# schmidtjonathan/Climate2Weather

Measured on AMD Instinct MI355X. Metric: UNet denoise steps/sec (train fwd+bwd+allreduce+AdamW+EMA windows/s), higher is better.
Workload: dtype bf16; 1 GPU; configs/sda_unet.yml default net, 5 vars x window 13 = 65 ch, 128x128, bf16 training step, 128 windows/GPU/step; global_batch=128, parallelism=dp1, params=72132929

## Files before the change

### climate2weather_amd/csrc/wgrad_patch.hip

```cpp
#include <algorithm>
#include <cstdint>
#include <cstdlib>
#include <utility>
#include "conv_geom.h"

#include "knobs.h"
#include "launch.h"


namespace {

constexpr int NTHREADS = 512;
constexpr int KPX = 128;
constexpr int ABYTES = KPX * 256;
constexpr int PPITCH = 24;
constexpr int NPIECE = 10 * 3;
constexpr int PBYTES = NPIECE * 1024;
constexpr int NSLOT_A = 3, NSLOT_P = 2;
constexpr int PBASE = NSLOT_A * ABYTES;
constexpr int LDS_BYTES = PBASE + NSLOT_P * PBYTES;

struct WpArgs {
    const void* dy;
    const void* x;
    float* dw;
    float* db;
    int B, H, W, Cin, Cout, ldy;
    int up;
    int ktiles, ktiles_per_split;
    float* ws;
    int direct;
    float* wsb;
    int det;
};

struct WpItem {
    const void* dy;
    const void* x;
    float* dw;
    float* db;
};
constexpr int WP_MAX_ITEMS = 16;
struct WpGroupArgs {
    WpArgs c;
    int n;
    int live_per_item;
    unsigned long long ws_item_floats;
    unsigned long long wsb_item_floats;
    WpItem item[WP_MAX_ITEMS];
};



__device__ __forceinline__ uint32_t sel_oob(bool ok, uint32_t v) {
    asm volatile("" : "+v"(v));
    return ok ? v : C2W_OOB;
}

__device__ __forceinline__ uint32_t swzA(int row) { return (uint32_t)(((row & 3) << 2) | ((row >> 2) & 3)); }
__device__ __forceinline__ uint32_t swzP(int pix) { return (uint32_t)((((pix >> 1) & 1) << 1) | (((pix >> 3) & 1) << 2)); }

__device__ __forceinline__ int wp_xcd_order(int bid, int nblk) {
    const int xcd = bid & 7, q = nblk >> 3, r = nblk & 7;
    return (xcd < r ? xcd * (q + 1) : r * (q + 1) + (xcd - r) * q) + (bid >> 3);
}

template <typename T, bool PAIR = false, bool NARROW = false>
__device__ __forceinline__ void wgrad_patch_body(const WpArgs& p, const int L) {
    constexpr int ESZ = sizeof(T);
    constexpr bool BF = ESZ == 2;
    constexpr int COT = 256 / ESZ;
    constexpr int CIB = 128 / ESZ;
    constexpr int MTW = BF ? 4 : 1;
    extern __shared__ __attribute__((aligned(16))) char smem[];

    const int tid = threadIdx.x, lane = tid & 63;
    const int wid = __builtin_amdgcn_readfirstlane(tid >> 6);
    const int li = lane & 15, lg = lane >> 4;
    static_assert(!NARROW || (BF && !PAIR), "narrow-M form: 16-bit, 16-pixel-wide tiles");
    const int mt0 = BF ? (NARROW ? (wid >> 2) * 4 : (wid & 1) * 4) : (wid >> 1);
    const int nt = BF ? (NARROW ? (wid & 3) : (wid >> 1)) : (wid & 1);
    const bool light = NARROW && wid >= 4;

    const int ncib = p.Cin / CIB;
    const int tilesM = (p.Cout + COT - 1) / COT;
    const int tilesMN = tilesM * ncib;
    const int split = L / tilesMN, mn = L - split * tilesMN;
    const int tm = mn / ncib, cb = mn - tm * ncib;
    const int co0 = tm * COT, ci0 = cb * CIB;
    const int H = p.H, W = p.W;
    const int tw = PAIR ? 1 : W >> 4, tpi = (H >> 3) * tw;
    const int t0 = split * p.ktiles_per_split;
    const int t1 = (t0 + p.ktiles_per_split < p.ktiles) ? t0 + p.ktiles_per_split : p.ktiles;

    const int Ws = p.up ? W >> 1 : W;
    const size_t ximg = (size_t)(p.up ? (H >> 1) * Ws : H * W) * p.Cin * ESZ;
    const size_t yimg = (size_t)H * W * p.ldy * ESZ;
    const uint32_t a_step = PAIR ? (uint32_t)(16 * p.ldy * ESZ) : (uint32_t)(2 * W * p.ldy * ESZ);
    auto dy_voff0 = [&](int tid_) -> uint32_t {
        const int row = tid_ >> 4, pc = tid_ & 15;
        const uint32_t lc = (uint32_t)pc ^ swzA(row);
        const int c = co0 + (int)lc * (16 / ESZ);
        if constexpr (PAIR) {
            return sel_oob(c < p.Cout, (uint32_t)((((row >> 4) * 8 + (row & 7)) * p.ldy + c) * ESZ) + (uint32_t)((row >> 3) & 1) * (uint32_t)yimg);
        } else {
            return sel_oob(c < p.Cout, (uint32_t)((((row >> 4) * W + (row & 15)) * p.ldy + c) * ESZ));
        }
    };
    auto patch_piece = [&](int r) -> int {
        const int pc = r * 8 + wid;
        return pc < NPIECE ? pc : NPIECE - 1;
    };
    auto patch_voff = [&](int r, int lane_, int oh0, int ow0) -> uint32_t {
        const int pc = patch_piece(r);
        const int pr = pc / 3, pg = pc - pr * 3;
        const int px = pg * 8 + (lane_ >> 3);
        const uint32_t lanepart = (uint32_t)(((lane_ & 7) ^ swzP(pr * PPITCH + px)) << 4) + (uint32_t)ci0 * ESZ;
        if constexpr (PAIR) {
            const int pimg = px >= 10 ? 1 : 0;
            const int ih = pr - 1, iw = px - 1 - 10 * pimg;
            const bool ok = (unsigned)ih < 8u && (unsigned)iw < 8u && px < 20;
            return sel_oob(ok, (uint32_t)((ih * 8 + iw) * p.Cin) * ESZ + (uint32_t)pimg * (uint32_t)(64 * p.Cin * ESZ) + lanepart);
        } else {
            const int ih = oh0 - 1 + pr, iw = ow0 - 1 + px;
            const bool ok = (unsigned)ih < (unsigned)H && (unsigned)iw < (unsigned)W && px < 18;
            const int spix = p.up ? (ih >> 1) * Ws + (iw >> 1) : ih * W + iw;
            return sel_oob(ok, (uint32_t)(spix * p.Cin) * ESZ + lanepart);
        }
    };

    auto tile_origin = [&](int t, int& b, int& oh0, int& ow0) {
        b = PAIR ? 2 * t : t / tpi;
        const int tt = PAIR ? 0 : t - (t / tpi) * tpi;
        const int ty = tt / tw, tx = tt - ty * tw;
        b = __builtin_amdgcn_readfirstlane(b);
        oh0 = __builtin_amdgcn_readfirstlane(ty << 3);
        ow0 = __builtin_amdgcn_readfirstlane(tx << 4);
    };
    struct TileSrc {
        __amdgpu_buffer_rsrc_t rsrc;
        int oh0, ow0;
        uint32_t aso;
        char* base;
    };
    auto srcA = [&](int t, int sa) {
        int b, oh0, ow0;
        tile_origin(t, b, oh0, ow0);
        const uint32_t nimg = PAIR && b + 1 < p.B ? 2u : 1u;
        TileSrc s;
        s.rsrc = make_rsrc((const char*)p.dy + (size_t)b * yimg, (uint32_t)yimg * nimg);
        s.oh0 = oh0;
        s.ow0 = ow0;
        s.aso = (uint32_t)((oh0 * W + ow0) * p.ldy) * ESZ;
        s.base = smem + sa * ABYTES + wid * 1024;
        return s;
    };
    auto srcP = [&](int t, int sp) {
        int b, oh0, ow0;
        tile_origin(t, b, oh0, ow0);
        const uint32_t nimg = PAIR && b + 1 < p.B ? 2u : 1u;
        TileSrc s;
        s.rsrc = make_rsrc((const char*)p.x + (size_t)b * ximg, (uint32_t)ximg * nimg);
        s.oh0 = oh0;
        s.ow0 = ow0;
        s.aso = 0;
        s.base = smem + PBASE + sp * PBYTES;
        return s;
    };
    auto pieceA = [&](const TileSrc& s, int i, bool live = true) {
        int tid_ = tid;
        asm volatile("" : "+v"(tid_));
        const uint32_t v = dy_voff0(tid_);
        glds16(s.rsrc, s.base + i * 8192, sel_oob(live, v), s.aso + (uint32_t)i * a_step);
    };
    auto pieceP = [&](const TileSrc& s, int r, bool live = true) {
        int lane_ = lane;
        asm volatile("" : "+v"(lane_));
        const uint32_t v = patch_voff(r, lane_, s.oh0, s.ow0);
        glds16(s.rsrc, s.base + patch_piece(r) * 1024, sel_oob(live, v), 0);
    };
    auto issueA = [&](int t, int sa) {
        const TileSrc s = srcA(t, sa);
#pragma unroll
        for (int i = 0; i < 4; ++i) pieceA(s, i);
    };
    auto issueP = [&](int t, int sp) {
        const TileSrc s = srcP(t, sp);
#pragma unroll
        for (int r = 0; r < 4; ++r) pieceP(s, r);
    };

    f32x4_t acc[9][MTW];
#pragma unroll
    for (int t = 0; t < 9; ++t)
#pragma unroll
        for (int m = 0; m < MTW; ++m) acc[t][m] = (f32x4_t){0.f, 0.f, 0.f, 0.f};
    const bool do_bias = p.db != nullptr && cb == 0 && nt == 0;
    f32x4_t accb[MTW];
#pragma unroll
    for (int m = 0; m < MTW; ++m) accb[m] = (f32x4_t){0.f, 0.f, 0.f, 0.f};

    uint32_t offA[MTW][2], offB[9][2];
    if constexpr (BF) {
        const int qq = li >> 2, pp = li & 3;
#pragma unroll
        for (int h = 0; h < 2; ++h) {
            const int row = 8 * lg + qq + 4 * h;
            const uint32_t f = swzA(row);
#pragma unroll
            for (int m = 0; m < MTW; ++m)
                offA[m][h] = (uint32_t)(row * 256 + (((((mt0 + m) * 2 + (pp >> 1)) ^ f) & 15) << 4) + 8 * (pp & 1));
            const int r = lg >> 1, c = 8 * (lg & 1) + qq + 4 * h;
#pragma unroll
            for (int t = 0; t < 9; ++t) {
                const int pix = (r + t / 3) * PPITCH + c + t % 3 + (PAIR ? 2 * (lg & 1) : 0);
                offB[t][h] = (uint32_t)(pix * 128 + (((uint32_t)(nt * 2 + (pp >> 1)) ^ swzP(pix)) << 4) + 8 * (pp & 1));
            }
        }
    }

    if (t0 < t1) {
        issueP(t0, 0);
        issueA(t0, 0);
        const TileSrc s1 = srcA(t0 + 1 < t1 ? t0 + 1 : t0, 1);
#pragma unroll
        for (int i = 0; i < 4; ++i) pieceA(s1, i, t0 + 1 < t1);
    }
    int sa = 0, sp = 0;
    for (int t = t0; t < t1; ++t) {
        asm volatile("s_waitcnt vmcnt(4)" ::: "memory");
        __builtin_amdgcn_s_barrier();
        const bool hasP = t + 1 < t1, hasA = t + 2 < t1;
        const TileSrc nP = srcP(hasP ? t + 1 : t, sp ^ 1), nA = srcA(hasA ? t + 2 : t, sa == 0 ? 2 : sa - 1);
        if constexpr (!BF) {
#pragma unroll
            for (int r = 0; r < 4; ++r) pieceP(nP, r, hasP);
#pragma unroll
            for (int i = 0; i < 4; ++i) pieceA(nA, i, hasA);
        }
        const char* const SA = smem + sa * ABYTES;
        const char* const SP = smem + PBASE + sp * PBYTES;
        if constexpr (BF) {
            const uint32_t sA = (uint32_t)(uintptr_t)SA, sP = (uint32_t)(uintptr_t)SP;
            auto rd = [&](tr_frag& f, uint32_t base, uint32_t o0, uint32_t o1, auto IMMc) {
                constexpr int IMM = decltype(IMMc)::value;
                asm volatile("ds_read_b64_tr_b16 %0, %1 offset:%2" : "=v"(f.lo) : "v"(base + o0), "n"(IMM));
                asm volatile("ds_read_b64_tr_b16 %0, %1 offset:%2" : "=v"(f.hi) : "v"(base + o1), "n"(IMM));
            };
            static_for<4>([&](auto KSc) {
                constexpr int ks = decltype(KSc)::value;
                {
                    const bool first = wid < 4;
                    if ((ks == 0 && first) || (ks == 1 && !first)) {
#pragma unroll
                        for (int r = 0; r < 4; ++r) pieceP(nP, r, hasP);
                    }
                    if ((ks == 2 && first) || (ks == 3 && !first)) {
#pragma unroll
                        for (int i = 0; i < 4; ++i) pieceA(nA, i, hasA);
                    }
                }
                constexpr int PF = 2;
                tr_frag a[MTW], bq[PF + 1];
                rd(a[0], sA, offA[0][0], offA[0][1], IC<ks * 32 * 256>{});
                if (!light) {
#pragma unroll
                    for (int m = 1; m < MTW; ++m) rd(a[m], sA, offA[m][0], offA[m][1], IC<ks * 32 * 256>{});
                }
                static_for<PF>([&](auto Jc) {
                    constexpr int j = decltype(Jc)::value;
                    rd(bq[j], sP, offB[j][0], offB[j][1], IC<ks * 2 * PPITCH * 128>{});
                });
                static_for<9>([&](auto TPc) {
                    constexpr int tp = decltype(TPc)::value;
                    if constexpr (tp + PF < 9) rd(bq[(tp + PF) % (PF + 1)], sP, offB[tp + PF][0], offB[tp + PF][1], IC<ks * 2 * PPITCH * 128>{});
                    constexpr int AHEAD = (tp + PF < 9 ? PF : 8 - tp) * 2;
                    if constexpr (AHEAD == 4) asm volatile("s_waitcnt lgkmcnt(4)" ::: "memory");
                    else if constexpr (AHEAD == 2) asm volatile("s_waitcnt lgkmcnt(2)" ::: "memory");
                    else asm volatile("s_waitcnt lgkmcnt(0)" ::: "memory");
                    __builtin_amdgcn_sched_barrier(0);
                    const bf16x8_t bfr = bq[tp % (PF + 1)].vec();
                    acc[tp][0] = mfma16s<T>(a[0].vec(), bfr, acc[tp][0]);
                    if (!light) {
#pragma unroll
                        for (int m = 1; m < MTW; ++m) acc[tp][m] = mfma16s<T>(a[m].vec(), bfr, acc[tp][m]);
                    }
                    if (tp == 8 && do_bias) {
                        const bf16x8_t ones = __builtin_bit_cast(bf16x8_t, ones16<T>());
                        accb[0] = mfma16s<T>(a[0].vec(), ones, accb[0]);
                        if (!light) {
#pragma unroll
                            for (int m = 1; m < MTW; ++m) accb[m] = mfma16s<T>(a[m].vec(), ones, accb[m]);
                        }
                    }
                    __builtin_amdgcn_sched_barrier(0);
                });
            });
        } else {
#pragma unroll 4
            for (int kk = 0; kk < 32; ++kk) {
                const int row = kk * 4 + lg;
                const float a = *(const float*)(SA + row * 256 + ((((uint32_t)(mt0 * 4 + (li >> 2))) ^ swzA(row)) << 4) + (li & 3) * 4);
                const int r = kk >> 2, c = 4 * (kk & 3) + lg;
#pragma unroll
                for (int tp = 0; tp < 9; ++tp) {
                    const int pix = (r + tp / 3) * PPITCH + c + tp % 3 + (PAIR && (kk & 2) ? 2 : 0);
                    const float bv = *(const float*)(SP + pix * 128 + ((((uint32_t)(nt * 4 + (li >> 2))) ^ swzP(pix)) << 4) + (li & 3) * 4);
                    acc[tp][0] = __builtin_amdgcn_mfma_f32_16x16x4f32(a, bv, acc[tp][0], 0, 0, 0);
                }
                if (do_bias) accb[0] = __builtin_amdgcn_mfma_f32_16x16x4f32(a, 1.0f, accb[0], 0, 0, 0);
            }
        }
        sa = sa == 2 ? 0 : sa + 1;
        sp ^= 1;
    }

    if (t0 >= t1) return;
    if (do_bias && li == 0) {
#pragma unroll
        for (int m = 0; m < MTW; ++m)
#pragma unroll
            for (int r = 0; r < 4; ++r) {
                const int row = (mt0 + m) * 16 + lg * 4 + r;
                const int co = co0 + row;
                if (p.det) {
                    if (p.wsb != nullptr) p.wsb[((size_t)split * tilesM + tm) * COT + row] = accb[m][r];
                    else if (co < p.Cout) p.db[co] = p.db[co] + accb[m][r];
                } else if (co < p.Cout) {
                    atomicAdd(p.db + co, accb[m][r]);
                }
            }
    }
    constexpr int OS = CIB + 4;
    float* const O = (float*)smem;
#pragma unroll
    for (int tp = 0; tp < 9; ++tp) {
        __syncthreads();
#pragma unroll
        for (int m = 0; m < MTW; ++m)
#pragma unroll
            for (int r = 0; r < 4; ++r) O[((mt0 + m) * 16 + lg * 4 + r) * OS + nt * 16 + li] = acc[tp][m][r];
        __syncthreads();
        if (p.ws != nullptr) {
            float* const dst = p.ws + (((size_t)split * tilesMN + mn) * 9 + tp) * (COT * CIB);
            for (int idx = tid; idx < COT * CIB; idx += NTHREADS) dst[idx] = O[(idx / CIB) * OS + (idx % CIB)];
        } else if (p.direct) {
            for (int idx = tid; idx < COT * CIB; idx += NTHREADS) {
                const int row = idx / CIB, col = idx - row * CIB;
                const int co = co0 + row;
                if (co < p.Cout) {
                    float* const d = p.dw + ((size_t)co * 9 + tp) * p.Cin + ci0 + col;
                    *d = *d + O[row * OS + col];
                }
            }
        } else {
            for (int idx = tid; idx < COT * CIB; idx += NTHREADS) {
                const int row = idx / CIB, col = idx - row * CIB;
                const int co = co0 + row;
                if (co < p.Cout) atomicAdd(p.dw + ((size_t)co * 9 + tp) * p.Cin + ci0 + col, O[row * OS + col]);
            }
        }
    }
}

template <typename T, bool PAIR = false, bool NARROW = false>
__global__ __launch_bounds__(NTHREADS, 2) void wgrad_patch_kernel(const WpArgs p) {
    wgrad_patch_body<T, PAIR, NARROW>(p, wp_xcd_order((int)blockIdx.x, (int)gridDim.x));
}

typedef __attribute__((address_space(4))) const char wp_kernarg_t;
__device__ __forceinline__ WpItem wp_item(int it) {
    const WpItem __attribute__((address_space(4)))* tab =
        (const WpItem __attribute__((address_space(4)))*)((wp_kernarg_t*)__builtin_amdgcn_kernarg_segment_ptr() + offsetof(WpGroupArgs, item));
    WpItem r;
    r.dy = tab[it].dy;
    r.x = tab[it].x;
    r.dw = tab[it].dw;
    r.db = tab[it].db;
    return r;
}

template <typename T, bool PAIR = false>
__global__ __launch_bounds__(NTHREADS, 2) void wgrad_patch_group_kernel(const WpGroupArgs g) {
    const int Lg = wp_xcd_order((int)blockIdx.x, (int)gridDim.x);
    const int it = __builtin_amdgcn_readfirstlane(Lg / g.live_per_item);
    const int L = Lg - it * g.live_per_item;
    const WpItem e = wp_item(it);
    WpArgs p = g.c;
    p.dy = e.dy;
    p.x = e.x;
    p.dw = e.dw;
    p.db = e.db;
    p.ws = g.c.ws != nullptr ? g.c.ws + (size_t)it * g.ws_item_floats : nullptr;
    p.wsb = g.c.wsb != nullptr ? g.c.wsb + (size_t)it * g.wsb_item_floats : nullptr;
    wgrad_patch_body<T, PAIR, false>(p, L);
}

struct WgradBiasReduce {
    const float* wsb;
    float* db;
    int cols, tpo, nmain;
};
static inline WgradBiasReduce bias_reduce_of(const float* wsb, float* db, int cols, int nsplit, int nmain) {
    WgradBiasReduce br;
    br.wsb = wsb; br.db = db; br.cols = cols; br.tpo = det_reduce_tpo(nsplit); br.nmain = nmain;
    return br;
}

#ifndef C2W_RED_COLS
#define C2W_RED_COLS 64
#endif
template <int COT, int CIB>
__device__ __forceinline__ void wgrad_reduce_body(const float* __restrict__ ws, float* __restrict__ dw, int nsplit, int tilesMN, int ncib,
                                                  int Cin, int Cout, int nblk) {
    constexpr int RC = C2W_RED_COLS, RG = 256 / RC;
    __shared__ f32x4_t red[RG][RC];
    const size_t per4 = (size_t)tilesMN * 9 * COT * CIB / 4;
    const f32x4_t* ws4 = (const f32x4_t*)ws;
    const int q = threadIdx.x % RC, grp = threadIdx.x / RC;
    for (size_t base = (size_t)blockIdx.x * RC; base < per4; base += (size_t)nblk * RC) {
        const size_t i4 = base + q;
        f32x4_t acc = {0.f, 0.f, 0.f, 0.f};
        if (i4 < per4) {
#pragma unroll 8
            for (int sidx = grp; sidx < nsplit; sidx += RG) acc += ws4[(size_t)sidx * per4 + i4];
        }
        red[grp][q] = acc;
        __syncthreads();
        if (grp == 0 && i4 < per4) {
#pragma unroll
            for (int g2 = 1; g2 < RG; ++g2) acc += red[g2][q];
            const size_t i = i4 * 4;
            const int col = (int)(i % CIB);
            size_t r = i / CIB;
            const int row = (int)(r % COT);
            r /= COT;
            const int tp = (int)(r % 9);
            const int mn = (int)(r / 9);
            const int tm = mn / ncib, cb = mn - tm * ncib;
            const int co = tm * COT + row;
            if (co < Cout) {
                f32x4_t* d = (f32x4_t*)(dw + ((size_t)co * 9 + tp) * Cin + cb * CIB + col);
                *d = *d + acc;
            }
        }
        __syncthreads();
    }
}

template <int COT, int CIB>
__global__ __launch_bounds__(256) void wgrad_reduce_kernel(const float* __restrict__ ws, float* __restrict__ dw, int nsplit, int tilesMN, int ncib,
                                                           int Cin, int Cout, WgradBiasReduce br) {
    if ((int)blockIdx.x >= br.nmain) {
        det_reduce_body(br.wsb, br.db, nsplit, Cout, Cout, 0, br.tpo, br.cols, (int)blockIdx.x - br.nmain);
        return;
    }
    wgrad_reduce_body<COT, CIB>(ws, dw, nsplit, tilesMN, ncib, Cin, Cout, br.nmain);
}
template <int COT, int CIB>
__global__ __launch_bounds__(256) void wgrad_reduce_group_kernel(const WpGroupArgs g, int nsplit, int tilesMN, int ncib, WgradBiasReduce br) {
    const int it = (int)blockIdx.y;
    const WpItem e = wp_item(it);
    if ((int)blockIdx.x >= br.nmain) {
        if (e.db != nullptr)
            det_reduce_body(g.c.wsb + (size_t)it * g.wsb_item_floats, e.db, nsplit, g.c.Cout, g.c.Cout, 0, br.tpo, br.cols, (int)blockIdx.x - br.nmain);
        return;
    }
    wgrad_reduce_body<COT, CIB>(g.c.ws + (size_t)it * g.ws_item_floats, e.dw, nsplit, tilesMN, ncib, g.c.Cin, g.c.Cout, br.nmain);
}

template <int ESZ, bool PAIR>
static void split_plan(const C2wConvArgs& a, int& ktiles, int& tilesMN, int& nsplit, int& ktiles_per_split) {
    constexpr int COT = 256 / ESZ, CIB = 128 / ESZ;
    ktiles = PAIR ? ((a.B + 1) >> 1) * (a.Hout >> 3) : a.B * (a.Hout >> 3) * (a.Wout >> 4);
    tilesMN = ((a.Cout + COT - 1) / COT) * (a.Cin / CIB);
    nsplit = c2w_cu_count() / tilesMN;
    if (nsplit > ktiles) nsplit = ktiles;
    if (nsplit < 1) nsplit = 1;
    ktiles_per_split = (ktiles + nsplit - 1) / nsplit;
    nsplit = (ktiles + ktiles_per_split - 1) / ktiles_per_split;
}

template <int ESZ, bool PAIR>
static size_t ws_need(const C2wConvArgs& a) {
    constexpr int COT = 256 / ESZ, CIB = 128 / ESZ;
    int ktiles, tilesMN, nsplit, per;
    split_plan<ESZ, PAIR>(a, ktiles, tilesMN, nsplit, per);
    const size_t bias_rows = (a.flags & C2W_CONV_DETERMINISTIC) ? (size_t)nsplit * ((a.Cout + COT - 1) / COT) * COT * sizeof(float) : 0;
    return nsplit > 1 ? (size_t)nsplit * tilesMN * 9 * COT * CIB * sizeof(float) + bias_rows : 0;
}

template <typename T, bool PAIR, bool NARROW = false>
int launch(const C2wConvArgs& a, float* dw, float* db, float* ws, size_t ws_bytes, hipStream_t st) {
    constexpr int ESZ = sizeof(T);
    constexpr int COT = 256 / ESZ, CIB = 128 / ESZ;
    WpArgs p;
    p.dy = a.y; p.x = a.x; p.dw = dw; p.db = db;
    p.B = a.B; p.H = a.Hout; p.W = a.Wout; p.Cin = a.Cin; p.Cout = a.Cout; p.ldy = a.ldy;
    p.up = a.mode == C2W_CONV_UP ? 1 : 0;
    int tilesMN, nsplit;
    split_plan<ESZ, PAIR>(a, p.ktiles, tilesMN, nsplit, p.ktiles_per_split);
    if (int rc = c2w_lds_optin<wgrad_patch_kernel<T, PAIR, NARROW>>(LDS_BYTES)) return rc;
    const size_t need = (size_t)nsplit * tilesMN * 9 * COT * CIB * sizeof(float);
    const int bias_cols = (tilesMN / (a.Cin / CIB)) * COT;
    p.det = (a.flags & C2W_CONV_DETERMINISTIC) ? 1 : 0;
    if (p.det) {
        if (c2w_knobs().wgrad_atomics) return C2W_ERR_BAD_ARG;
        if (nsplit > 1 && (ws == nullptr || need + (size_t)nsplit * bias_cols * sizeof(float) > ws_bytes)) return C2W_ERR_BAD_ARG;
    }
    p.ws = (ws != nullptr && need <= ws_bytes && nsplit > 1 && !c2w_knobs().wgrad_atomics) ? ws : nullptr;
    p.wsb = p.det && nsplit > 1 && db != nullptr ? ws + need / sizeof(float) : nullptr;
    p.direct = nsplit == 1 && !c2w_knobs().wgrad_atomics ? 1 : 0;
    wgrad_patch_kernel<T, PAIR, NARROW><<<tilesMN * nsplit, NTHREADS, LDS_BYTES, st>>>(p);
    if (p.ws != nullptr) {
        const size_t per_split = (size_t)tilesMN * 9 * COT * CIB;
        const int grid = (int)std::min<size_t>((per_split / 4 + C2W_RED_COLS - 1) / C2W_RED_COLS, 8192);
        const int extra = p.wsb != nullptr ? det_reduce_blocks(nsplit, a.Cout) : 0;
        wgrad_reduce_kernel<COT, CIB><<<grid + extra, 256, 0, st>>>(p.ws, dw, nsplit, tilesMN, a.Cin / CIB, a.Cin, a.Cout,
                                                                    bias_reduce_of(p.wsb, db, bias_cols, nsplit, grid));
    }
    return (int)hipGetLastError();
}

static void group_plan(int n, int tilesMN, int ktiles, int& nsplit, int& ktiles_per_split) {
    const int T = n * tilesMN, cus = c2w_cu_count();
    double best = 1e30;
    nsplit = 1;
    for (int r = 0; r <= 4; ++r) {
        int ns = r == 0 ? 1 : (cus * r) / T;
        if (ns < 1) ns = 1;
        if (ns > ktiles) ns = ktiles;
        const int per = (ktiles + ns - 1) / ns;
        ns = (ktiles + per - 1) / per;
        const int rounds = (T * ns + cus - 1) / cus;
        const double cost = rounds * (per * 4.1 + (ns > 1 ? 28.0 : 16.0)) + (ns > 1 ? 10.0 : 0.0);
        if (cost < best - 1e-9) {
            best = cost;
            nsplit = ns;
        }
    }
    ktiles_per_split = (ktiles + nsplit - 1) / nsplit;
}

template <int ESZ, bool PAIR>
static size_t group_ws_need(const C2wConvArgs& a, int n) {
    constexpr int COT = 256 / ESZ, CIB = 128 / ESZ;
    int ktiles, tilesMN, ns1, per1, nsplit, per;
    split_plan<ESZ, PAIR>(a, ktiles, tilesMN, ns1, per1);
    group_plan(n, tilesMN, ktiles, nsplit, per);
    const size_t bias_rows = (a.flags & C2W_CONV_DETERMINISTIC) ? (size_t)n * nsplit * ((a.Cout + COT - 1) / COT) * COT * sizeof(float) : 0;
    return nsplit > 1 ? (size_t)n * nsplit * tilesMN * 9 * COT * CIB * sizeof(float) + bias_rows : 0;
}

template <typename T, bool PAIR>
int launch_group(const C2wConvArgs& a, const C2wWgradItem* items, int n, float* ws, size_t ws_bytes, hipStream_t st) {
    constexpr int ESZ = sizeof(T);
    constexpr int COT = 256 / ESZ, CIB = 128 / ESZ;
    WpGroupArgs g;
    WpArgs& p = g.c;
    p.dy = nullptr; p.x = nullptr; p.dw = nullptr; p.db = nullptr;
    p.B = a.B; p.H = a.Hout; p.W = a.Wout; p.Cin = a.Cin; p.Cout = a.Cout; p.ldy = a.ldy;
    p.up = a.mode == C2W_CONV_UP ? 1 : 0;
    int tilesMN, ns1, per1, nsplit;
    split_plan<ESZ, PAIR>(a, p.ktiles, tilesMN, ns1, per1);
    group_plan(n, tilesMN, p.ktiles, nsplit, p.ktiles_per_split);
    const size_t item_floats = (size_t)nsplit * tilesMN * 9 * COT * CIB;
    const int bias_cols = (tilesMN / (a.Cin / CIB)) * COT;
    p.det = (a.flags & C2W_CONV_DETERMINISTIC) ? 1 : 0;
    const size_t bias_item_floats = p.det ? (size_t)nsplit * bias_cols : 0;
    if (nsplit > 1 && (ws == nullptr || (size_t)n * (item_floats + bias_item_floats) * sizeof(float) > ws_bytes)) return C2W_ERR_BAD_ARG;
    p.ws = nsplit > 1 ? ws : nullptr;
    p.wsb = p.det && nsplit > 1 ? ws + (size_t)n * item_floats : nullptr;
    g.wsb_item_floats = bias_item_floats;
    p.direct = nsplit == 1 ? 1 : 0;
    g.n = n;
    g.live_per_item = tilesMN * nsplit;
    g.ws_item_floats = item_floats;
    for (int i = 0; i < WP_MAX_ITEMS; ++i) {
        const C2wWgradItem& e = items[i < n ? i : n - 1];
        g.item[i].dy = e.dy; g.item[i].x = e.x; g.item[i].dw = e.dw; g.item[i].db = e.dbias;
    }
    if (int rc = c2w_lds_optin<wgrad_patch_group_kernel<T, PAIR>>(LDS_BYTES)) return rc;
    wgrad_patch_group_kernel<T, PAIR><<<g.live_per_item * n, NTHREADS, LDS_BYTES, st>>>(g);
    if (p.ws != nullptr) {
        const size_t per_split = (size_t)tilesMN * 9 * COT * CIB;
        const int grid = (int)std::min<size_t>((per_split / 4 + C2W_RED_COLS - 1) / C2W_RED_COLS, 8192);
        const int extra = p.wsb != nullptr ? det_reduce_blocks(nsplit, a.Cout) : 0;
        wgrad_reduce_group_kernel<COT, CIB><<<dim3(grid + extra, n), 256, 0, st>>>(g, nsplit, tilesMN, a.Cin / CIB,
                                                                                   bias_reduce_of(p.wsb, nullptr, bias_cols, nsplit, grid));
    }
    return (int)hipGetLastError();
}

}

bool c2w_wgrad_patch_group_eligible(const C2wConvArgs& a, int n, int dtype) {
    const bool narrow = dtype != C2W_DTYPE_F32 && !c2w_wgrad_patch_pair(a) && a.Cout <= 80;
    return c2w_wgrad_patch_eligible(a) && n >= 2 && n <= WP_MAX_ITEMS && !narrow && !c2w_knobs().wgrad_atomics;
}

int c2w_wgrad_patch_group(const C2wConvArgs& a, const C2wWgradItem* items, int n, float* ws, size_t ws_bytes, int dtype, hipStream_t st) {
    if (c2w_wgrad_patch_pair(a)) return c2w_by_dtype(dtype, [&](auto t) { return launch_group<decltype(t), true>(a, items, n, ws, ws_bytes, st); });
    return c2w_by_dtype(dtype, [&](auto t) { return launch_group<decltype(t), false>(a, items, n, ws, ws_bytes, st); });
}

size_t c2w_wgrad_patch_group_ws_bytes(const C2wConvArgs& a, int n, int dtype) {
    const bool pair = c2w_wgrad_patch_pair(a);
    if (dtype == C2W_DTYPE_F32) return pair ? group_ws_need<4, true>(a, n) : group_ws_need<4, false>(a, n);
    return pair ? group_ws_need<2, true>(a, n) : group_ws_need<2, false>(a, n);
}

bool c2w_wgrad_patch_pair(const C2wConvArgs& a) {
    return a.mode == C2W_CONV_S1 && a.Win == 8 && a.Hin == 8;
}

bool c2w_wgrad_patch_eligible(const C2wConvArgs& a) {
    if (a.mode == C2W_CONV_UP)
        return a.Hout == 2 * a.Hin && a.Wout == 2 * a.Win && (a.Hout & 7) == 0 && (a.Wout & 15) == 0;
    return a.mode == C2W_CONV_S1 && a.Hin == a.Hout && a.Win == a.Wout && (a.Hin & 7) == 0 && ((a.Win & 15) == 0 || c2w_wgrad_patch_pair(a));
}

int c2w_wgrad_patch(const C2wConvArgs& a, float* dw, float* db, float* ws, size_t ws_bytes, int dtype, hipStream_t st) {
    if (c2w_wgrad_patch_pair(a)) return c2w_by_dtype(dtype, [&](auto t) { return launch<decltype(t), true>(a, dw, db, ws, ws_bytes, st); });
    if (dtype != C2W_DTYPE_F32 && a.Cout <= 80)
        return c2w_by_dtype16(dtype, [&](auto t) { return launch<decltype(t), false, true>(a, dw, db, ws, ws_bytes, st); });
    return c2w_by_dtype(dtype, [&](auto t) { return launch<decltype(t), false>(a, dw, db, ws, ws_bytes, st); });
}

size_t c2w_wgrad_patch_ws_bytes(const C2wConvArgs& a, int dtype) {
    const bool pair = c2w_wgrad_patch_pair(a);
    if (dtype == C2W_DTYPE_F32) return pair ? ws_need<4, true>(a) : ws_need<4, false>(a);
    return pair ? ws_need<2, true>(a) : ws_need<2, false>(a);
}
```

Baseline: 2802 windows/s.

## Spread wgrad bias MFMAs across waves and add flat split-K reduce path

Moves bias-gradient accumulation off a single wave. Each wave in the bf16 path now computes at most one 16-row bias tile, and the M-tile order is rotated per wave so that different waves own different tiles. The light path zeros the unused wsb rows. A second, independent change adds a grid-stride flat reduction kernel for split-K workspaces when nsplit is at most 32. It uses several independent accumulators and a smaller grid sized from the CU count, replacing the column-block reduce body. Risks are wrong bias coverage if the ownership mapping misses tiles, and lower parallelism in the reduce for large outputs.

After: 2824 windows/s, median of 6. No clear change (+0.8%).

```diff
diff --git a/climate2weather_amd/csrc/wgrad_patch.hip b/climate2weather_amd/csrc/wgrad_patch.hip
--- a/climate2weather_amd/csrc/wgrad_patch.hip
+++ b/climate2weather_amd/csrc/wgrad_patch.hip
@@ -195,10 +195,16 @@
     for (int t = 0; t < 9; ++t)
 #pragma unroll
         for (int m = 0; m < MTW; ++m) acc[t][m] = (f32x4_t){0.f, 0.f, 0.f, 0.f};
-    const bool do_bias = p.db != nullptr && cb == 0 && nt == 0;
-    f32x4_t accb[MTW];
-#pragma unroll
-    for (int m = 0; m < MTW; ++m) accb[m] = (f32x4_t){0.f, 0.f, 0.f, 0.f};
+    const int rot = BF && !light ? nt : 0;
+    auto tile_of = [&](int m) { return mt0 + ((m + rot) & (MTW - 1)); };
+    int bm = -1;
+    if (p.db != nullptr) {
+        const int half2 = ncib >= 2 ? 1 : 0;
+        if constexpr (!BF) bm = cb == 0 && nt == 0 ? 0 : -1;
+        else if (light) bm = cb == half2 && nt == 0 ? 0 : -1;
+        else bm = cb == (half2 ? nt >> 1 : 0) ? nt : -1;
+    }
+    f32x4_t accb = (f32x4_t){0.f, 0.f, 0.f, 0.f};
 
     uint32_t offA[MTW][2], offB[9][2];
     if constexpr (BF) {
@@ -209,7 +215,7 @@
             const uint32_t f = swzA(row);
 #pragma unroll
             for (int m = 0; m < MTW; ++m)
-                offA[m][h] = (uint32_t)(row * 256 + (((((mt0 + m) * 2 + (pp >> 1)) ^ f) & 15) << 4) + 8 * (pp & 1));
+                offA[m][h] = (uint32_t)(row * 256 + ((((tile_of(m) * 2 + (pp >> 1)) ^ f) & 15) << 4) + 8 * (pp & 1));
             const int r = lg >> 1, c = 8 * (lg & 1) + qq + 4 * h;
 #pragma unroll
             for (int t = 0; t < 9; ++t) {
@@ -285,13 +291,9 @@
 #pragma unroll
                         for (int m = 1; m < MTW; ++m) acc[tp][m] = mfma16s<T>(a[m].vec(), bfr, acc[tp][m]);
                     }
-                    if (tp == 8 && do_bias) {
+                    if (tp == 8 && bm >= 0) {
                         const bf16x8_t ones = __builtin_bit_cast(bf16x8_t, ones16<T>());
-                        accb[0] = mfma16s<T>(a[0].vec(), ones, accb[0]);
-                        if (!light) {
-#pragma unroll
-                            for (int m = 1; m < MTW; ++m) accb[m] = mfma16s<T>(a[m].vec(), ones, accb[m]);
-                        }
+                        accb = mfma16s<T>(a[0].vec(), ones, accb);
                     }
                     __builtin_amdgcn_sched_barrier(0);
                 });
@@ -308,7 +310,7 @@
                     const float bv = *(const float*)(SP + pix * 128 + ((((uint32_t)(nt * 4 + (li >> 2))) ^ swzP(pix)) << 4) + (li & 3) * 4);
                     acc[tp][0] = __builtin_amdgcn_mfma_f32_16x16x4f32(a, bv, acc[tp][0], 0, 0, 0);
                 }
-                if (do_bias) accb[0] = __builtin_amdgcn_mfma_f32_16x16x4f32(a, 1.0f, accb[0], 0, 0, 0);
+                if (bm >= 0) accb = __builtin_amdgcn_mfma_f32_16x16x4f32(a, 1.0f, accb, 0, 0, 0);
             }
         }
         sa = sa == 2 ? 0 : sa + 1;
@@ -316,20 +318,24 @@
     }
 
     if (t0 >= t1) return;
-    if (do_bias && li == 0) {
-#pragma unroll
-        for (int m = 0; m < MTW; ++m)
-#pragma unroll
-            for (int r = 0; r < 4; ++r) {
-                const int row = (mt0 + m) * 16 + lg * 4 + r;
-                const int co = co0 + row;
-                if (p.det) {
-                    if (p.wsb != nullptr) p.wsb[((size_t)split * tilesM + tm) * COT + row] = accb[m][r];
-                    else if (co < p.Cout) p.db[co] = p.db[co] + accb[m][r];
-                } else if (co < p.Cout) {
-                    atomicAdd(p.db + co, accb[m][r]);
-                }
+    if (bm >= 0 && li == 0) {
+#pragma unroll
+        for (int r = 0; r < 4; ++r) {
+            const int row = (mt0 + bm) * 16 + lg * 4 + r;
+            const int co = co0 + row;
+            if (p.det) {
+                if (p.wsb != nullptr) p.wsb[((size_t)split * tilesM + tm) * COT + row] = accb[r];
+                else if (co < p.Cout) p.db[co] = p.db[co] + accb[r];
+            } else if (co < p.Cout) {
+                atomicAdd(p.db + co, accb[r]);
             }
+        }
+        if (light && p.det && p.wsb != nullptr) {
+#pragma unroll
+            for (int i = 16; i < 64; i += 16)
+#pragma unroll
+                for (int r = 0; r < 4; ++r) p.wsb[((size_t)split * tilesM + tm) * COT + mt0 * 16 + i + lg * 4 + r] = 0.f;
+        }
     }
     constexpr int OS = CIB + 4;
     float* const O = (float*)smem;
@@ -339,7 +345,7 @@
 #pragma unroll
         for (int m = 0; m < MTW; ++m)
 #pragma unroll
-            for (int r = 0; r < 4; ++r) O[((mt0 + m) * 16 + lg * 4 + r) * OS + nt * 16 + li] = acc[tp][m][r];
+            for (int r = 0; r < 4; ++r) O[(tile_of(m) * 16 + lg * 4 + r) * OS + nt * 16 + li] = acc[tp][m][r];
         __syncthreads();
         if (p.ws != nullptr) {
             float* const dst = p.ws + (((size_t)split * tilesMN + mn) * 9 + tp) * (COT * CIB);
@@ -448,6 +454,55 @@
     }
 }
 
+#ifndef C2W_RED_FLAT_MAX
+#define C2W_RED_FLAT_MAX 32
+#endif
+template <int COT, int CIB>
+__device__ __forceinline__ void wgrad_reduce_flat_body(const float* __restrict__ ws, float* __restrict__ dw, int nsplit, int tilesMN, int ncib,
+                                                       int Cin, int Cout, int nblk) {
+    constexpr int RG = 256 / C2W_RED_COLS;
+    const size_t per4 = (size_t)tilesMN * 9 * COT * CIB / 4;
+    const f32x4_t* ws4 = (const f32x4_t*)ws;
+    for (size_t i4 = (size_t)blockIdx.x * 256 + threadIdx.x; i4 < per4; i4 += (size_t)nblk * 256) {
+        f32x4_t a[RG];
+#pragma unroll
+        for (int g = 0; g < RG; ++g) a[g] = (f32x4_t){0.f, 0.f, 0.f, 0.f};
+        const f32x4_t* s = ws4 + i4;
+        int k = 0;
+#pragma unroll 2
+        for (; k + RG <= nsplit; k += RG) {
+#pragma unroll
+            for (int g = 0; g < RG; ++g) a[g] += s[(size_t)(k + g) * per4];
+        }
+#pragma unroll
+        for (int g = 0; g < RG - 1; ++g)
+            if (k + g < nsplit) a[g] += s[(size_t)(k + g) * per4];
+        f32x4_t acc = a[0];
+#pragma unroll
+        for (int g = 1; g < RG; ++g) acc += a[g];
+        const size_t i = i4 * 4;
+        const int col = (int)(i % CIB);
+        size_t r = i / CIB;
+        const int row = (int)(r % COT);
+        r /= COT;
+        const int tp = (int)(r % 9);
+        const int mn = (int)(r / 9);
+        const int tm = mn / ncib, cb = mn - tm * ncib;
+        const int co = tm * COT + row;
+        if (co < Cout) {
+            f32x4_t* d = (f32x4_t*)(dw + ((size_t)co * 9 + tp) * Cin + cb * CIB + col);
+            *d = *d + acc;
+        }
+    }
+}
+static inline int reduce_grid(size_t per_split_floats, int nsplit, int n) {
+    if (nsplit <= C2W_RED_FLAT_MAX) {
+        const size_t all = (per_split_floats / 4 + 255) / 256, few = (size_t)std::max(1, 8 * c2w_cu_count() / n);
+        return (int)std::min(all, few);
+    }
+    return (int)std::min<size_t>((per_split_floats / 4 + C2W_RED_COLS - 1) / C2W_RED_COLS, 8192);
+}
+
 template <int COT, int CIB>
 __global__ __launch_bounds__(256) void wgrad_reduce_kernel(const float* __restrict__ ws, float* __restrict__ dw, int nsplit, int tilesMN, int ncib,
                                                            int Cin, int Cout, WgradBiasReduce br) {
@@ -455,7 +510,8 @@
         det_reduce_body(br.wsb, br.db, nsplit, Cout, Cout, 0, br.tpo, br.cols, (int)blockIdx.x - br.nmain);
         return;
     }
-    wgrad_reduce_body<COT, CIB>(ws, dw, nsplit, tilesMN, ncib, Cin, Cout, br.nmain);
+    if (nsplit <= C2W_RED_FLAT_MAX) wgrad_reduce_flat_body<COT, CIB>(ws, dw, nsplit, tilesMN, ncib, Cin, Cout, br.nmain);
+    else wgrad_reduce_body<COT, CIB>(ws, dw, nsplit, tilesMN, ncib, Cin, Cout, br.nmain);
 }
 template <int COT, int CIB>
 __global__ __launch_bounds__(256) void wgrad_reduce_group_kernel(const WpGroupArgs g, int nsplit, int tilesMN, int ncib, WgradBiasReduce br) {
@@ -466,7 +522,9 @@
             det_reduce_body(g.c.wsb + (size_t)it * g.wsb_item_floats, e.db, nsplit, g.c.Cout, g.c.Cout, 0, br.tpo, br.cols, (int)blockIdx.x - br.nmain);
         return;
     }
-    wgrad_reduce_body<COT, CIB>(g.c.ws + (size_t)it * g.ws_item_floats, e.dw, nsplit, tilesMN, ncib, g.c.Cin, g.c.Cout, br.nmain);
+    const float* const ws = g.c.ws + (size_t)it * g.ws_item_floats;
+    if (nsplit <= C2W_RED_FLAT_MAX) wgrad_reduce_flat_body<COT, CIB>(ws, e.dw, nsplit, tilesMN, ncib, g.c.Cin, g.c.Cout, br.nmain);
+    else wgrad_reduce_body<COT, CIB>(ws, e.dw, nsplit, tilesMN, ncib, g.c.Cin, g.c.Cout, br.nmain);
 }
 
 template <int ESZ, bool PAIR>
@@ -514,7 +572,7 @@
     wgrad_patch_kernel<T, PAIR, NARROW><<<tilesMN * nsplit, NTHREADS, LDS_BYTES, st>>>(p);
     if (p.ws != nullptr) {
         const size_t per_split = (size_t)tilesMN * 9 * COT * CIB;
-        const int grid = (int)std::min<size_t>((per_split / 4 + C2W_RED_COLS - 1) / C2W_RED_COLS, 8192);
+        const int grid = reduce_grid(per_split, nsplit, 1);
         const int extra = p.wsb != nullptr ? det_reduce_blocks(nsplit, a.Cout) : 0;
         wgrad_reduce_kernel<COT, CIB><<<grid + extra, 256, 0, st>>>(p.ws, dw, nsplit, tilesMN, a.Cin / CIB, a.Cin, a.Cout,
                                                                     bias_reduce_of(p.wsb, db, bias_cols, nsplit, grid));
@@ -584,7 +642,7 @@
     wgrad_patch_group_kernel<T, PAIR><<<g.live_per_item * n, NTHREADS, LDS_BYTES, st>>>(g);
     if (p.ws != nullptr) {
         const size_t per_split = (size_t)tilesMN * 9 * COT * CIB;
-        const int grid = (int)std::min<size_t>((per_split / 4 + C2W_RED_COLS - 1) / C2W_RED_COLS, 8192);
+        const int grid = reduce_grid(per_split, nsplit, n);
         const int extra = p.wsb != nullptr ? det_reduce_blocks(nsplit, a.Cout) : 0;
         wgrad_reduce_group_kernel<COT, CIB><<<dim3(grid + extra, n), 256, 0, st>>>(g, nsplit, tilesMN, a.Cin / CIB,
                                                                                    bias_reduce_of(p.wsb, nullptr, bias_cols, nsplit, grid));
```
